# NoliNobdon/TriStage-RAG

Hardware: AMD Instinct MI355X
Metric: end-to-end queries/sec @10Mx768 corpus (stage-1 exact top-k, pre-encoded HBM-resident queries) (higher is better)
Workload: dtype f16; 1 GPU; synthetic 10000000x768 f16 corpus, batch-64 queries, stage-1 exact top-1000, row-sharded over 1 GPU(s); rows=10000000, dim=768, batch=64, k=1000, submission=batches enqueued back to back (async), verified by finish() in the timed region, max_candidates_per_query=6027

## Files before the change

include/tristage.h:

```cpp
#ifndef TRISTAGE_H_
#define TRISTAGE_H_

#include <stdint.h>

#ifdef __cplusplus
extern "C" {
#endif

#define TS_ABI_VERSION 4

typedef struct ts_index ts_index;

enum ts_status {
  TS_OK = 0,
  TS_ERR_INVALID = -1,
  TS_ERR_HIP = -2,
  TS_ERR_OOM = -3,
  TS_ERR_EMPTY = -4,
  TS_ERR_UNSUPPORTED = -5
};

enum ts_dtype { TS_F32 = 0, TS_F16 = 1, TS_BF16 = 2,
               TS_FP8_E4M3 = 3  };

enum ts_metric { TS_METRIC_INNER_PRODUCT = 0 };

#define TS_FLAG_HOST_PTR 1u
#define TS_FLAG_NO_FILTER 2u
#define TS_FLAG_ASYNC 8u
#define TS_FLAG_PIPELINE 16u
#define TS_FLAG_CLASSIC 32u
#define TS_FLAG_ONE_LAUNCH 64u
#define TS_FLAG_COALESCE 128u
#define TS_FLAG_WIDE_PASSES 256u
#define TS_FLAG_NO_WIDE_PASSES 512u
#define TS_FLAG_NORMALIZE 4u

int ts_index_create(int32_t dim, int32_t storage_dtype, int32_t metric,
                    int32_t device, ts_index** out);
int ts_index_destroy(ts_index* h);
int ts_index_reset(ts_index* h);
int ts_index_reserve(ts_index* h, int64_t nrows);

int ts_index_add(ts_index* h, const void* rows, int64_t n, int32_t rows_dtype,
                 uint32_t flags, void* stream);

int ts_index_search(ts_index* h, const void* queries, int32_t nq,
                    int32_t q_dtype, int32_t k, float* out_scores,
                    int64_t* out_ids, uint32_t flags, void* stream);

int ts_index_search_filtered(ts_index* h, const void* queries, int32_t nq, int32_t q_dtype, int32_t k,
                             const uint32_t* allow_bits, int64_t allow_words, int32_t n_masks,
                             const int32_t* mask_of_query, float* out_scores, int64_t* out_ids,
                             uint32_t flags, void* stream);
int ts_index_last_filter_info(const ts_index* h, int64_t info[4]);

int ts_index_range_search(ts_index* h, const void* queries, int32_t nq, int32_t q_dtype, const float* radius,
                          const uint32_t* allow_bits, int64_t allow_words, int32_t n_masks,
                          const int32_t* mask_of_query, int64_t max_total, int64_t* lims, uint32_t flags,
                          void* stream);
int ts_index_range_fetch(ts_index* h, float* out_scores, int64_t* out_ids, int64_t capacity, uint32_t flags,
                         void* stream);

int ts_index_scores(ts_index* h, const void* queries, int32_t nq, int32_t q_dtype,
                    float* out, int64_t ld, void* stream);

int64_t ts_index_last_ticket(const ts_index* h);
int ts_index_filter_path(const ts_index* h, int32_t k);
int ts_index_finish(ts_index* h, void* stream, int64_t* failed_tickets, int32_t max_failed,
                    int32_t* n_failed);

int ts_index_flush(ts_index* h, void* stream);
int32_t ts_coalesce_groups(int32_t dim, int32_t storage_dtype);
int32_t ts_coalesce_groups_wide(int32_t dim, int32_t storage_dtype);
int64_t ts_coalesce_wide_min_bytes(void);

int ts_index_remove(ts_index* h, const int64_t* ids, int64_t n, int64_t* n_removed, void* stream);
int64_t ts_index_live_count(const ts_index* h);
int ts_index_live_words(ts_index* h, uint32_t* out, void* stream);
int ts_index_compact(ts_index* h, int64_t* old2new, void* stream);

int ts_index_update(ts_index* h, const int64_t* ids, int64_t n, const void* rows, int32_t rows_dtype,
                    uint32_t flags, void* stream);

int64_t ts_index_ntotal(const ts_index* h);
int32_t ts_index_dim(const ts_index* h);
int32_t ts_index_dtype(const ts_index* h);

int ts_index_set_fp8_scale_log2(ts_index* h, int32_t s);
int32_t ts_index_fp8_scale_log2(const ts_index* h);
int ts_index_mmr(ts_index* h, const int64_t* cand_ids, const float* cand_rel, int32_t nq, int32_t fetch_k, int32_t k,
                 float lambda, float* out_rel, int64_t* out_ids, uint32_t flags, void* stream);
int ts_index_mmr_set_timing(ts_index* h, int32_t on);
int ts_index_mmr_get_timings(ts_index* h, double ms[3], int64_t* calls, int32_t reset);
int ts_index_search_prefix(ts_index* h, const void* queries, int32_t nq, int32_t q_dtype, int32_t dims, int32_t k,
                           const uint32_t* allow_bits, int64_t allow_words, int32_t n_masks,
                           const int32_t* mask_of_query, float* out_scores, int64_t* out_ids, uint32_t flags,
                           void* hip_stream);
int ts_index_rescore(ts_index* h, const void* queries, int32_t nq, int32_t q_dtype, const int64_t* cand_ids,
                     int32_t ncand, int32_t k, float* out_scores, int64_t* out_ids, void* hip_stream);
int ts_index_set_id_offset(ts_index* h, int64_t offset);
int ts_index_reconstruct(ts_index* h, int64_t row0, int64_t n, float* out,
                         uint32_t flags, void* stream);
int ts_index_last_search_info(const ts_index* h, int64_t info[4]);

int ts_index_set_profiling(ts_index* h, int32_t on);
int ts_index_get_timings(ts_index* h, double ms[8], int64_t counts[8], int32_t reset);

// ... 142 lines not shown
```

tristage-rag_amd/_lib.py:

```python
from __future__ import annotations

import ctypes
import os
import subprocess
from ctypes import POINTER, c_char_p, c_float, c_int32, c_int64, c_uint32, c_void_p

_HERE = os.path.dirname(os.path.abspath(__file__))
LIB_PATH = os.environ.get("TRISTAGE_LIB") or os.path.join(_HERE, "libtristage.so")
CSRC_DIR = os.path.join(_HERE, "csrc")

TS_OK = 0
TS_ERR_INVALID, TS_ERR_HIP, TS_ERR_OOM, TS_ERR_EMPTY, TS_ERR_UNSUPPORTED = -1, -2, -3, -4, -5
TS_F32, TS_F16, TS_BF16, TS_FP8_E4M3 = 0, 1, 2, 3
TS_METRIC_INNER_PRODUCT = 0
HEADER_PATH = os.path.join(os.path.dirname(_HERE), "include", "tristage.h")


def header_abi_version() -> int:
    import re
    m = re.search(r"^#define\s+TS_ABI_VERSION\s+(\d+)", open(HEADER_PATH).read(), flags=re.M)
    if not m:
        raise ImportError(f"TS_ABI_VERSION not found in {HEADER_PATH}")
    return int(m.group(1))


TS_FLAG_HOST_PTR, TS_FLAG_NO_FILTER, TS_FLAG_NORMALIZE, TS_FLAG_ASYNC, TS_FLAG_PIPELINE, TS_FLAG_CLASSIC, TS_FLAG_ONE_LAUNCH = 1, 2, 4, 8, 16, 32, 64
TS_FLAG_COALESCE = 128
TS_FLAG_WIDE_PASSES, TS_FLAG_NO_WIDE_PASSES = 256, 512

SIGNATURES = {
    "ts_index_create": (c_int32, [c_int32, c_int32, c_int32, c_int32, POINTER(c_void_p)]),
    "ts_index_destroy": (c_int32, [c_void_p]),
    "ts_index_reset": (c_int32, [c_void_p]),
    "ts_index_reserve": (c_int32, [c_void_p, c_int64]),
    "ts_index_add": (c_int32, [c_void_p, c_void_p, c_int64, c_int32, c_uint32, c_void_p]),
    "ts_index_search": (c_int32, [c_void_p, c_void_p, c_int32, c_int32, c_int32, c_void_p,
                                  c_void_p, c_uint32, c_void_p]),
    "ts_index_search_filtered": (c_int32, [c_void_p, c_void_p, c_int32, c_int32, c_int32, c_void_p, c_int64, c_int32,
                                           c_void_p, c_void_p, c_void_p, c_uint32, c_void_p]),
    "ts_index_last_filter_info": (c_int32, [c_void_p, POINTER(c_int64)]),
    "ts_index_range_search": (c_int32, [c_void_p, c_void_p, c_int32, c_int32, c_void_p, c_void_p, c_int64, c_int32,
                                        c_void_p, c_int64, c_void_p, c_uint32, c_void_p]),
    "ts_index_range_fetch": (c_int32, [c_void_p, c_void_p, c_void_p, c_int64, c_uint32, c_void_p]),
    "ts_index_scores": (c_int32, [c_void_p, c_void_p, c_int32, c_int32, c_void_p, c_int64, c_void_p]),
    "ts_index_remove": (c_int32, [c_void_p, c_void_p, c_int64, POINTER(c_int64), c_void_p]),
    "ts_index_update": (c_int32, [c_void_p, c_void_p, c_int64, c_void_p, c_int32, c_uint32, c_void_p]),
    "ts_index_live_count": (c_int64, [c_void_p]),
    "ts_index_live_words": (c_int32, [c_void_p, c_void_p, c_void_p]),
    "ts_index_compact": (c_int32, [c_void_p, c_void_p, c_void_p]),
    "ts_index_ntotal": (c_int64, [c_void_p]),
    "ts_index_dim": (c_int32, [c_void_p]),
    "ts_index_dtype": (c_int32, [c_void_p]),
    "ts_index_set_fp8_scale_log2": (c_int32, [c_void_p, c_int32]),
    "ts_index_fp8_scale_log2": (c_int32, [c_void_p]),
    "ts_index_set_id_offset": (c_int32, [c_void_p, c_int64]),
    "ts_index_reconstruct": (c_int32, [c_void_p, c_int64, c_int64, c_void_p, c_uint32, c_void_p]),
    "ts_index_last_search_info": (c_int32, [c_void_p, POINTER(c_int64)]),
    "ts_index_last_ticket": (c_int64, [c_void_p]),
    "ts_index_filter_path": (c_int32, [c_void_p, c_int32]),
    "ts_index_finish": (c_int32, [c_void_p, c_void_p, POINTER(c_int64), c_int32, POINTER(c_int32)]),
    "ts_index_flush": (c_int32, [c_void_p, c_void_p]),
    "ts_coalesce_groups": (c_int32, [c_int32, c_int32]),
    "ts_coalesce_groups_wide": (c_int32, [c_int32, c_int32]),
    "ts_coalesce_wide_min_bytes": (c_int64, []),
    "ts_index_set_profiling": (c_int32, [c_void_p, c_int32]),
    "ts_index_get_timings": (c_int32, [c_void_p, POINTER(ctypes.c_double), POINTER(c_int64), c_int32]),
    "ts_index_read_probe": (c_int32, [c_void_p, c_int32, POINTER(ctypes.c_double), POINTER(ctypes.c_double),
                                      POINTER(c_int64), c_void_p]),
    "ts_ivf_create": (c_int32, [c_int32, c_int32, c_int32, c_int32, POINTER(c_void_p)]),
    "ts_ivf_destroy": (c_int32, [c_void_p]),
    "ts_ivf_reset": (c_int32, [c_void_p]),
    "ts_ivf_train": (c_int32, [c_void_p, c_void_p, c_int64, c_int32, c_int64, c_int32, c_void_p, c_void_p]),
    "ts_ivf_set_centroids": (c_int32, [c_void_p, c_void_p, c_void_p]),
    "ts_ivf_get_centroids": (c_int32, [c_void_p, c_void_p, c_void_p]),
    "ts_ivf_is_trained": (c_int32, [c_void_p]),
    "ts_ivf_add": (c_int32, [c_void_p, c_void_p, c_int64, c_int32, c_uint32, c_void_p]),
    "ts_ivf_search": (c_int32, [c_void_p, c_void_p, c_int32, c_int32, c_int32, c_int32, c_void_p, c_void_p, c_void_p]),
    "ts_ivf_probe": (c_int32, [c_void_p, c_void_p, c_int32, c_int32, c_int32, c_void_p, c_void_p, c_void_p]),
    "ts_ivf_list_sizes": (c_int32, [c_void_p, c_void_p]),
    "ts_ivf_reconstruct": (c_int32, [c_void_p, c_int64, c_int64, c_void_p, c_void_p]),
    "ts_ivf_ntotal": (c_int64, [c_void_p]),
    "ts_remove_ivf": (c_int32, [c_void_p, c_void_p, c_int64, POINTER(c_int64), c_void_p]),
    "ts_update_ivf": (c_int32, [c_void_p, c_void_p, c_int64, c_void_p, c_int32, c_uint32, c_void_p]),
    "ts_compact_ivf": (c_int32, [c_void_p, c_void_p, c_void_p]),
    "ts_index_mmr": (c_int32, [c_void_p, c_void_p, c_void_p, c_int32, c_int32, c_int32, c_float, c_void_p, c_void_p,
                               c_uint32, c_void_p]),
    "ts_index_search_prefix": (c_int32, [c_void_p, c_void_p, c_int32, c_int32, c_int32, c_int32, c_void_p, c_int64, c_int32,
                                         c_void_p, c_void_p, c_void_p, c_uint32, c_void_p]),
    "ts_index_rescore": (c_int32, [c_void_p, c_void_p, c_int32, c_int32, c_void_p, c_int32, c_int32, c_void_p, c_void_p,
                                   c_void_p]),
    "ts_index_mmr_set_timing": (c_int32, [c_void_p, c_int32]),
    "ts_index_mmr_get_timings": (c_int32, [c_void_p, POINTER(ctypes.c_double), POINTER(c_int64), c_int32]),
    "ts_mmr_ivf": (c_int32, [c_void_p, c_void_p, c_void_p, c_int32, c_int32, c_int32, c_float, c_void_p, c_void_p,
                             c_uint32, c_void_p]),
    "ts_ivf_set_id_offset": (c_int32, [c_void_p, c_int64]),
    "ts_ivf_last_search_info": (c_int32, [c_void_p, POINTER(c_int64)]),
# ... 108 lines not shown
```

tristage-rag_amd/csrc/ts_common.h:

```cpp
#pragma once
#include <hip/hip_runtime.h>
#include <stdint.h>
#include <stddef.h>

#include "../../include/tristage.h"

void ts_set_error(const char* fmt, ...);

#define TS_HIP(call)                                                        \
  do {                                                                      \
    hipError_t e_ = (call);                                                 \
    if (e_ != hipSuccess) {                                                 \
      ts_set_error("%s failed: %s (%s:%d)", #call, hipGetErrorString(e_),   \
                   __FILE__, __LINE__);                                     \
      return (e_ == hipErrorOutOfMemory) ? TS_ERR_OOM : TS_ERR_HIP;         \
    }                                                                       \
  } while (0)

#define TS_CHECK(call)            \
  do {                            \
    int s_ = (call);              \
    if (s_ != TS_OK) return s_;   \
  } while (0)

// ... 102 lines not shown
                                 hipStream_t stream);

#define TS_MAX_GROUPS 4
struct MultiScanParams : ScanParams {
  const uint4* gimg[TS_MAX_GROUPS];
  int gqh[TS_MAX_GROUPS];
  int ghalf[TS_MAX_GROUPS];
  const float* gtau[TS_MAX_GROUPS];
  uint32_t* gcnt[TS_MAX_GROUPS];
  float* gscore[TS_MAX_GROUPS];
  int32_t* gid[TS_MAX_GROUPS];
  uint32_t stage_cap;
};
int ts_scan_multi_groups(const TsLayout& L);
uint32_t ts_scan_multi_stage_cap(const TsLayout& L, int G);
bool ts_scan_multi_fits(int64_t nblk, int num_cus);
int ts_launch_scan_multi(const TsLayout& L, int G, const MultiScanParams& p, int num_cus, hipStream_t stream);

#define TS_MAX_WIDE_GROUPS 8
struct WideScanParams : ScanParams {
  const uint4* gimg[TS_MAX_WIDE_GROUPS];
  int gqh[TS_MAX_WIDE_GROUPS];
  int ghalf[TS_MAX_WIDE_GROUPS];
  const float* gtau[TS_MAX_WIDE_GROUPS];
  uint32_t* gcnt[TS_MAX_WIDE_GROUPS];
  float* gscore[TS_MAX_WIDE_GROUPS];
  int32_t* gid[TS_MAX_WIDE_GROUPS];
  uint32_t stage_cap;
};
int ts_scan_wide_groups(const TsLayout& L);
uint32_t ts_scan_wide_stage_cap(const TsLayout& L, int G);
bool ts_scan_wide_fits(int64_t nblk, int num_cus);
int ts_launch_scan_wide(const TsLayout& L, int G, const WideScanParams& p, int num_cus, hipStream_t stream);

struct MultiTombParams : MultiScanParams {
  const uint32_t* live;
};
struct WideTombParams : WideScanParams {
  const uint32_t* live;
};
int ts_launch_scan_multi_tomb(const TsLayout& L, int G, const MultiTombParams& p, int num_cus, hipStream_t stream);
int ts_launch_scan_wide_tomb(const TsLayout& L, int G, const WideTombParams& p, int num_cus, hipStream_t stream);

int ts_launch_scan(const TsLayout& L, int mode, int qh, const ScanParams& p,
                   int num_cus, hipStream_t stream);

struct TsMaskPass {
  int32_t nd;
  int32_t all_live;
  int32_t dist[TS_MAX_Q];
  int32_t qmask[TS_MAX_Q];
  int32_t qd[TS_MAX_Q];
};
struct TsMaskDev {
  int32_t qmask[TS_MAX_Q];
  int32_t qd[TS_MAX_Q];
  uint32_t popc[TS_MAX_Q];
  uint32_t need[TS_MAX_Q];
  uint32_t nlive;
  uint32_t pad[63];
};
int ts_launch_live_blocks(const uint32_t* bits, int64_t words, const TsMaskPass& mp, int64_t nblk,
                          int64_t ntotal, TsMaskDev* md, hipStream_t stream);
int ts_launch_tau_masked(const float* sample, int64_t S, int64_t sstride, int64_t ntotal, const uint32_t* bits,
                         int64_t words, TsMaskDev* md, int nq, int k, uint32_t over, uint32_t min_rank,
                         float* tau, uint32_t* report, hipStream_t stream);
// ... 214 lines not shown
```

tristage-rag_amd/csrc/ts_index.hip:

```cpp
#include <stdarg.h>
#include <stdio.h>
#include <string.h>
#include <stdlib.h>

#include <algorithm>
#include <atomic>
#include <condition_variable>
#include <mutex>
#include <new>
#include <thread>
#include <vector>

#include "ts_common.h"

static thread_local char g_err[512] = "";

void ts_set_error(const char* fmt, ...) {
  va_list ap;
  va_start(ap, fmt);
  vsnprintf(g_err, sizeof(g_err), fmt, ap);
  va_end(ap);
}

extern "C" const char* ts_last_error(void) { return g_err; }
// ... 32 lines not shown
    b.p = nullptr;
    ts_set_error("hipMalloc(%zu bytes) failed: %s", want, hipGetErrorString(e));
    return TS_ERR_OOM;
  }
  b.bytes = want;
  return TS_OK;
}

void release(DevBuf& b) {
  if (b.p) (void)hipFree(b.p);
  b.p = nullptr;
  b.bytes = 0;
}

}
#define TS_NPHASE 8
#define TS_NSETS 8
#define TS_ASYNC_SLOTS 1024
#define TS_SLOT_WORDS 80
namespace {
constexpr int64_t kMinFilterRows = 32768;
constexpr int kMaxFilterK = 2048;
constexpr uint32_t kCandCap = 16384;
constexpr int64_t kMinSampleRows = 8192;
constexpr int64_t kSampleDiv = 128;
constexpr uint32_t kMinSampleRank = 24;
constexpr uint32_t kOversample = 4;
constexpr int64_t kDenseChunkRows = 1 << 20;
constexpr int64_t kOneLaunchMaxRows = 4 << 20;
constexpr int kHeadStartUs = 12;
constexpr int64_t kCoalesceOversample = 3;
constexpr int64_t kWideMinCorpusBytes = 256ll << 20;
constexpr int kWideMaxResidentGroups = 3;

}

struct ts_index {
  int device = 0;
  int num_cus = 256;
  TsLayout L{};
  int64_t ntotal = 0;
  int64_t cap_blocks = 0;
  uint4* corpus = nullptr;
  int64_t id_offset = 0;
  int64_t info[4] = {0, 0, 0, 0};
  int64_t finfo[4] = {0, 0, 0, 0};
  int64_t fseq = 0;
  struct WSet {
    DevBuf qimg, small, cand_score, cand_id, sample;
    DevBuf dense, list_score, list_id;
    DevBuf hist, spill;
    DevBuf mask, mids;
    uint32_t gen = 0;
    uint32_t arrive_total = 0;
    bool hist_dirty = false;
    unsigned long long* tau64() { return (unsigned long long*)((char*)small.p + 1024); }
    uint32_t* arrive() { return (uint32_t*)((char*)small.p + 2048); }
    hipEvent_t ev_pro = nullptr, ev_scan = nullptr, ev_sel = nullptr, ev_in = nullptr;
    bool used = false;
    bool busy = false;
    float* tau() { return (float*)small.p; }
    uint32_t* cand_cnt() { return (uint32_t*)small.p + 64; }
    uint32_t* status() { return (uint32_t*)small.p + 128; }
  };
  WSet ws[TS_NSETS];
  uint64_t set_next = 0;
  std::mutex mu;
  std::condition_variable cv;
  std::mutex host_mu;
  std::mutex prof_mu;
  bool slot_busy[TS_ASYNC_SLOTS] = {};
  hipStream_t s_pro = nullptr, s_scan = nullptr, s_sel = nullptr;
  DevBuf stage, den, qstage, out_s, out_i, mstage;
  uint32_t* host_status = nullptr;
  uint32_t* host_status_dev = nullptr;
  struct Pending { int64_t ticket; int slot; int nq; uint32_t S; uint32_t m; hipEvent_t e0, e1; int set; int64_t fseq; };
  Pending pending[TS_ASYNC_SLOTS];
  int npending = 0;
  uint64_t slot_next = 0;
  int64_t next_ticket = 0;
  hipEvent_t async_ev[2 * TS_ASYNC_SLOTS] = {};
  struct CoBatch { WSet* W; int nq, qh, k, slot, groups_left; float* out_s; int64_t* out_i; };
  struct CoGroup { int batch, half; };
  std::mutex co_mu;
  int co_gmax = 0;
  int co_gwide = 0;
  int co_width = 0;
  hipStream_t co_stream = nullptr;
  CoBatch co_batch[TS_MAX_WIDE_GROUPS] = {};
  int co_nbatch = 0;
  CoGroup co_group[TS_MAX_WIDE_GROUPS] = {};
  int co_ngroup = 0;
  uint64_t co_pass_seq = 0;
  hipEvent_t co_ev = nullptr;
  bool co_ev_live = false;
  bool profiling = false;
  int prof_every = 1;
  std::atomic<uint64_t> prof_seq{0};
  hipEvent_t ev[TS_NPHASE + 1] = {};
  double phase_ms[TS_NPHASE] = {};
  int64_t phase_cnt[TS_NPHASE] = {};
  DevBuf live;
  int64_t live_cap_words = 0;
  int64_t nremoved = 0;
  DevBuf eff, rids, compact_scratch, compact_stage;
  DevBuf upd_tile, upd_tab;
  std::mutex eff_mu;
  hipEvent_t eff_ev = nullptr;
  bool eff_used = false;
  DevBuf rng_s, rng_i, rng_tiles;
  int64_t rng_cap = 0, rng_total = 0;
  bool rng_valid = false;
  std::mutex range_mu;
  TsMmrWork mmr;
  DevBuf rescore_scratch;
  std::mutex rescore_mu;
};

static int co_flush(ts_index* h, hipStream_t s);

// ... 53 lines not shown
                               int32_t device, ts_index** out) {
  if (!out) { ts_set_error("out is null"); return TS_ERR_INVALID; }
  *out = nullptr;
  if (dim <= 0 || dim > 65536) { ts_set_error("bad dim %d", dim); return TS_ERR_INVALID; }
  if (storage_dtype != TS_F32 && storage_dtype != TS_F16 && storage_dtype != TS_BF16 &&
      storage_dtype != TS_FP8_E4M3) {
    ts_set_error("bad storage dtype %d", storage_dtype);
    return TS_ERR_INVALID;
  }
  if (metric != TS_METRIC_INNER_PRODUCT) {
    ts_set_error("only the inner-product metric is supported (reference uses IndexFlatIP)");
    return TS_ERR_UNSUPPORTED;
  }
  int ndev = 0;
  TS_HIP(hipGetDeviceCount(&ndev));
  if (device < 0 || device >= ndev) {
    ts_set_error("device %d not present (%d HIP devices)", device, ndev);
    return TS_ERR_INVALID;
  }
  TsLayout L = ts_make_layout(dim, storage_dtype);
  if (ts_scan_lds_bytes(L, 1) > 160 * 1024) {
    ts_set_error("dim %d with dtype %d needs %zu bytes of LDS for 32 queries (max 163840)", dim,
                 storage_dtype, ts_scan_lds_bytes(L, 1));
    return TS_ERR_UNSUPPORTED;
  }
  DeviceGuard g(device);
  if (!g.ok) { ts_set_error("hipSetDevice(%d) failed", device); return TS_ERR_HIP; }
  ts_index* h = new (std::nothrow) ts_index();
  if (!h) { ts_set_error("out of host memory"); return TS_ERR_OOM; }
  h->device = device;
  h->L = L;
  h->co_gmax = ts_coalesce_groups(dim, storage_dtype);
  h->co_gwide = ts_coalesce_groups_wide(dim, storage_dtype);
  hipDeviceProp_t prop;
  if (hipGetDeviceProperties(&prop, device) == hipSuccess && prop.multiProcessorCount > 0)
    h->num_cus = prop.multiProcessorCount;
  int st = TS_OK;
  for (ts_index::WSet& w : h->ws) {
    if (st == TS_OK) st = ensure(w.small, 4096);
    if (st == TS_OK && hipMemset(w.small.p, 0, 4096) != hipSuccess) { ts_set_error("hipMemset failed"); st = TS_ERR_HIP; }
    if (st == TS_OK) st = ensure(w.qimg, (size_t)L.qkg * 2 * 1024);
    if (st == TS_OK && (hipEventCreateWithFlags(&w.ev_pro, hipEventDisableTiming) != hipSuccess ||
                        hipEventCreateWithFlags(&w.ev_scan, hipEventDisableTiming) != hipSuccess ||
                        hipEventCreateWithFlags(&w.ev_sel, hipEventDisableTiming) != hipSuccess ||
                        hipEventCreateWithFlags(&w.ev_in, hipEventDisableTiming) != hipSuccess)) {
      ts_set_error("hipEventCreate failed");
      st = TS_ERR_HIP;
    }
  }
  if (st == TS_OK && hipStreamSynchronize(nullptr) != hipSuccess) { ts_set_error("hipStreamSynchronize failed"); st = TS_ERR_HIP; }
  if (st == TS_OK && (hipEventCreateWithFlags(&h->co_ev, hipEventDisableTiming) != hipSuccess ||
                      hipEventCreateWithFlags(&h->eff_ev, hipEventDisableTiming) != hipSuccess)) {
    ts_set_error("hipEventCreate failed");
    st = TS_ERR_HIP;
  }
  if (st == TS_OK &&
      (hipHostMalloc((void**)&h->host_status, (size_t)(TS_ASYNC_SLOTS + 1) * TS_SLOT_WORDS * 4, hipHostMallocMapped) != hipSuccess ||
       hipHostGetDevicePointer((void**)&h->host_status_dev, h->host_status, 0) != hipSuccess)) {
    ts_set_error("hipHostMalloc(mapped) failed");
    st = TS_ERR_HIP;
  }
  if (st != TS_OK) {
    ts_index_destroy(h);
    return st;
  }
  *out = h;
  return TS_OK;
}

extern "C" int ts_index_destroy(ts_index* h) {
// ... 676 lines not shown
  TS_HIP(hipStreamSynchronize(s));
  prof_collect(h, pc);
  uint32_t maxc = 0;
  for (int i = 0; i < nq; ++i) maxc = std::max(maxc, rep[i]);
  const bool redo = rep[64] != 0;
  set_info(h, (redo ? 2 : 1) | (fused ? 16 : 0), maxc, S, m);
  if (mc) add_filter_info(h, fseq, rep[65], nblk, false);
  if (redo) {
    if (fused) {
      W.hist_dirty = true;
      TS_CHECK(ts_launch_qprep(h->L, dq, q_dtype, nq, qh, (uint4*)W.qimg.p, W.cand_cnt(), W.status(), s));
    }
    prof_mark(h, pc, 5, s);
    TS_CHECK(dense_path(h, W, nq, qh, k, out_s, out_i, s, mc, pkg));
    prof_mark(h, pc, -1, s);
    TS_HIP(hipStreamSynchronize(s));
    prof_collect(h, pc);
  }
  return TS_OK;
}

extern "C" int32_t ts_coalesce_groups(int32_t dim, int32_t storage_dtype) {
  if (dim <= 0 || (storage_dtype != TS_F16 && storage_dtype != TS_BF16)) return 0;
  return ts_scan_multi_groups(ts_make_layout(dim, storage_dtype));
}

extern "C" int32_t ts_coalesce_groups_wide(int32_t dim, int32_t storage_dtype) {
  if (dim <= 0 || (storage_dtype != TS_F16 && storage_dtype != TS_BF16)) return 0;
  return ts_scan_wide_groups(ts_make_layout(dim, storage_dtype));
}

extern "C" int64_t ts_coalesce_wide_min_bytes() { return kWideMinCorpusBytes; }

static int co_pass_width(const ts_index* h, int k, uint32_t flags) {
  const int64_t N = h->ntotal;
  const int64_t nblk = (N + TS_ROWS_PER_BLOCK - 1) / TS_ROWS_PER_BLOCK;
  const uint32_t need = TS_FLAG_ASYNC | TS_FLAG_COALESCE;
  if ((flags & need) != need || (flags & (TS_FLAG_PIPELINE | TS_FLAG_NO_FILTER | TS_FLAG_HOST_PTR | TS_FLAG_ONE_LAUNCH)))
    return 0;
  if (k > kMaxFilterK || N < kMinFilterRows || N < 32 * (int64_t)k) return 0;
  if (!(flags & TS_FLAG_CLASSIC) && N <= kOneLaunchMaxRows) return 0;
  const int grid = h->num_cus - h->num_cus / 8;
  bool wide = (int64_t)nblk * (int64_t)ts_block_bytes(h->L) > kWideMinCorpusBytes &&
              h->co_gmax <= kWideMaxResidentGroups;
  if (flags & TS_FLAG_WIDE_PASSES) wide = true;
  if (flags & TS_FLAG_NO_WIDE_PASSES) wide = false;
  if (wide && h->co_gwide >= 3 && ts_scan_wide_fits(nblk, h->num_cus)) return h->co_gwide;
  if (h->co_gmax >= 3 && ts_scan_multi_fits(nblk, grid)) return h->co_gmax;
  return 0;
}

template <class P>
static void co_fill_params(const ts_index* h, int G, P& mp) {
  const int64_t N = h->ntotal;
  mp.corpus = h->corpus;
  mp.kg = h->L.kg;
  mp.nwork = (N + TS_ROWS_PER_BLOCK - 1) / TS_ROWS_PER_BLOCK;
  mp.blk0 = 0;
  mp.blk_stride = 1;
  mp.ntotal = N;
  mp.cand_cap = kCandCap;
  for (int g = 0; g < G; ++g) {
    const ts_index::CoBatch& b = h->co_batch[h->co_group[g].batch];
    const int half = h->co_group[g].half;
    mp.gimg[g] = (const uint4*)b.W->qimg.p;
    mp.gqh[g] = b.qh;
    mp.ghalf[g] = half;
    mp.gtau[g] = b.W->tau() + 32 * half;
    mp.gcnt[g] = b.W->cand_cnt() + 32 * half;
    mp.gscore[g] = (float*)b.W->cand_score.p + (size_t)32 * half * kCandCap;
    mp.gid[g] = (int32_t*)b.W->cand_id.p + (size_t)32 * half * kCandCap;
  }
}

static int co_launch_pass(ts_index* h) {
  if (h->co_ngroup == 0) return TS_OK;
  const int G = h->co_ngroup;
  const int64_t N = h->ntotal;
  hipStream_t s = h->co_stream;
  hipEvent_t e0 = nullptr, e1 = nullptr;
  if (h->profiling && h->co_pass_seq++ % (uint64_t)h->prof_every == 0) {
    if (hipEventCreate(&e0) != hipSuccess || hipEventCreate(&e1) != hipSuccess || hipEventRecord(e0, s) != hipSuccess) {
      if (e0) (void)hipEventDestroy(e0);
      if (e1) (void)hipEventDestroy(e1);
      e0 = e1 = nullptr;
    }
  }
  int st;
  const bool tomb = h->nremoved > 0;
  if (G <= h->co_gmax) {
    MultiTombParams mp{};
    co_fill_params(h, G, mp);
    mp.stage_cap = ts_scan_multi_stage_cap(h->L, G);
    mp.live = (const uint32_t*)h->live.p;
    st = tomb ? ts_launch_scan_multi_tomb(h->L, G, mp, h->num_cus - h->num_cus / 8, s)
              : ts_launch_scan_multi(h->L, G, mp, h->num_cus - h->num_cus / 8, s);
  } else {
    WideTombParams wp{};
    co_fill_params(h, G, wp);
    wp.stage_cap = ts_scan_wide_stage_cap(h->L, G);
    wp.live = (const uint32_t*)h->live.p;
    int wide_cus = h->num_cus;
#ifdef TS_TUNING
    static const int dbg_wide_cus = getenv("TS_WIDE_CUS") ? atoi(getenv("TS_WIDE_CUS")) : 0;
    if (dbg_wide_cus > 0) wide_cus = dbg_wide_cus;
#endif
    st = tomb ? ts_launch_scan_wide_tomb(h->L, G, wp, wide_cus, s) : ts_launch_scan_wide(h->L, G, wp, wide_cus, s);
  }
  if (e0 && (st != TS_OK || hipEventRecord(e1, s) != hipSuccess)) {
    (void)hipEventDestroy(e0);
    (void)hipEventDestroy(e1);
    e0 = e1 = nullptr;
  }
  for (int g = 0; g < G; ++g) --h->co_batch[h->co_group[g].batch].groups_left;
  h->co_ngroup = 0;
  int keep = 0;
  const int nb = h->co_nbatch;
  for (int i = 0; i < nb; ++i) {
    ts_index::CoBatch b = h->co_batch[i];
    if (b.groups_left > 0) { h->co_batch[keep++] = b; continue; }
    if (st == TS_OK) {
      SelParams p{};
      p.mode = SEL_PAIRS32;
// ... 156 lines not shown
    std::vector<int32_t> moq((size_t)nq, -1);
    return ts_index_search_filtered(h, queries, nq, q_dtype, k, nullptr, 0, 0, moq.data(), out_scores, out_ids, flags,
                                    stream);
  }
  DeviceGuard g(h->device);
  hipStream_t s = (hipStream_t)stream;
  const int qp = (ts_scan_lds_bytes(h->L, 2) <= 160 * 1024) ? 64 : 32;
  if ((flags & TS_FLAG_PIPELINE) && !(flags & TS_FLAG_ASYNC)) {
    ts_set_error("TS_FLAG_PIPELINE needs TS_FLAG_ASYNC");
    return TS_ERR_INVALID;
  }
  if (flags & TS_FLAG_ASYNC) {
    if (flags & TS_FLAG_HOST_PTR) { ts_set_error("TS_FLAG_ASYNC needs device pointers"); return TS_ERR_INVALID; }
    const int passes = (nq + qp - 1) / qp;
    if (passes > 4) { ts_set_error("TS_FLAG_ASYNC: at most %d queries per call", 4 * qp); return TS_ERR_INVALID; }
    bool full = false;
    {
      std::lock_guard<std::mutex> lk(h->mu);
      full = h->npending + passes > TS_ASYNC_SLOTS / 4;
    }
    if (full) {
      (void)co_flush(h, s);
      ts_set_error("too many unfinished asynchronous searches; call ts_index_finish()");
      return TS_ERR_INVALID;
    }
  }
  const size_t qrow = (size_t)h->L.dim * dtype_size(q_dtype);
  if (const int width = co_pass_width(h, k, flags)) {
    std::lock_guard<std::mutex> lk(h->co_mu);
    if (h->co_stream != s) TS_CHECK(co_flush_locked(h, s));
    if (h->co_ngroup > 0 && h->co_width != width) TS_CHECK(co_flush_locked(h, s));
    h->co_stream = s;
    h->co_width = width;
    for (int q0 = 0; q0 < nq; q0 += qp) {
      const int c = std::min(qp, nq - q0);
      TS_CHECK(co_submit(h, (const char*)queries + (size_t)q0 * qrow, c, q_dtype, k, out_scores + (size_t)q0 * k,
                         out_ids + (size_t)q0 * k, s));
    }
    std::lock_guard<std::mutex> lk2(h->mu);
    ++h->next_ticket;
    return TS_OK;
  }
  TS_CHECK(co_flush(h, s));
  const void* dq = queries;
  float* ds = out_scores;
  int64_t* di = out_ids;
  const bool host = (flags & TS_FLAG_HOST_PTR) != 0;
  std::unique_lock<std::mutex> hlk(h->host_mu, std::defer_lock);
  if (host) {
    hlk.lock();
    TS_CHECK(ensure(h->qstage, (size_t)nq * qrow));
    TS_CHECK(ensure(h->out_s, (size_t)nq * k * 4));
    TS_CHECK(ensure(h->out_i, (size_t)nq * k * 8));
    TS_HIP(hipMemcpyAsync(h->qstage.p, queries, (size_t)nq * qrow, hipMemcpyHostToDevice, s));
    dq = h->qstage.p;
    ds = (float*)h->out_s.p;
    di = (int64_t*)h->out_i.p;
  }
  for (int q0 = 0; q0 < nq; q0 += qp) {
    const int c = std::min(qp, nq - q0);
    TS_CHECK(search_pass(h, (const char*)dq + (size_t)q0 * qrow, c, q_dtype, k,
                         ds + (size_t)q0 * k, di + (size_t)q0 * k, flags, s));
  }
  if (flags & TS_FLAG_ASYNC) {
    std::lock_guard<std::mutex> lk(h->mu);
    ++h->next_ticket;
// ... 1319 lines not shown
```

tristage-rag_amd/index.py:

```python
from __future__ import annotations

import ctypes
from typing import NamedTuple, Optional

import numpy as np

from . import _lib

_NP_DTYPES = {np.dtype(np.float32): _lib.TS_F32, np.dtype(np.float16): _lib.TS_F16}
_NAME_TO_DTYPE = {"f32": _lib.TS_F32, "fp32": _lib.TS_F32, "float32": _lib.TS_F32,
                  "f16": _lib.TS_F16, "fp16": _lib.TS_F16, "float16": _lib.TS_F16,
                  "bf16": _lib.TS_BF16, "bfloat16": _lib.TS_BF16,
                  "fp8": _lib.TS_FP8_E4M3, "e4m3": _lib.TS_FP8_E4M3, "float8_e4m3fn": _lib.TS_FP8_E4M3}
_DTYPE_NAME = {_lib.TS_F32: "f32", _lib.TS_F16: "f16", _lib.TS_BF16: "bf16", _lib.TS_FP8_E4M3: "fp8"}
FP8_INDEX_MAX_D = 2048


def _torch():
    import torch
    return torch


def _is_tensor(x) -> bool:
    return type(x).__module__.startswith("torch") and hasattr(x, "data_ptr")
# ... 15 lines not shown
        mask = mask.detach().cpu().numpy()
    m = np.asarray(mask)
    words = (int(n) + 31) // 32
    if m.dtype == np.bool_:
        if m.ndim != 1 or m.shape[0] != n:
            raise ValueError(f"a bool allow mask must have one entry per row ({n}), got shape {m.shape}")
        b = np.packbits(m, bitorder="little")
        out = np.zeros(words * 4, dtype=np.uint8)
        out[: b.shape[0]] = b
        return out.view("<u4").astype(np.uint32)
    if m.dtype in (np.uint32, np.int32):
        if m.ndim != 1 or m.shape[0] < words:
            raise ValueError(f"a packed allow mask needs >= {words} uint32 words, got shape {m.shape}")
        w = np.ascontiguousarray(m[:words]).view(np.uint32).copy()
        if n % 32:
            w[-1] &= np.uint32((1 << (n % 32)) - 1)
        return w
    raise TypeError(f"allow mask: expected a bool array or packed uint32 words, got dtype {m.dtype}")


def _stream_ptr(device_index: int) -> int:
    torch = _torch()
    return int(torch.cuda.current_stream(device_index).cuda_stream)


def wide_pass_flags(wide_passes) -> int:
    if wide_passes is True:
        return _lib.TS_FLAG_WIDE_PASSES
    if wide_passes is False:
        return _lib.TS_FLAG_NO_WIDE_PASSES
    if isinstance(wide_passes, str) and wide_passes == "auto":
        return 0
    raise ValueError(f"wide_passes must be 'auto', True or False, not {wide_passes!r}")


def _addr(x) -> Optional[int]:
    if x is None:
        return None
    return x.data_ptr() if _is_tensor(x) else x.ctypes.data


def _raise_empty():
    raise ValueError("No documents indexed. Call add_documents() first.")


def _check(code: int, invalid: bool = False) -> None:
    if code == _lib.TS_ERR_EMPTY:
        _raise_empty()
    if invalid and code == _lib.TS_ERR_INVALID:
        raise ValueError(_lib.last_error())
    _lib.check(code)



def _bad_shape(n, d: int, what: str, shape):
    raise ValueError(f"expected [{n}, {d}] {what}, got {tuple(shape)}")


def _host_query(x, d: int, what: str = "queries", n="B", device: Optional[int] = None):
    if _is_tensor(x) and not x.is_cuda:
        x = x.detach().float().numpy()
    on_gpu = _is_tensor(x)
    if not on_gpu:
        x = np.ascontiguousarray(x)
        if x.dtype not in _NP_DTYPES:
            x = x.astype(np.float32)
# ... 307 lines not shown

    supports_out = True
    PENDING_PASSES = 240
    MAX_KERNEL_K = 16384
    MAX_ASYNC_QUERIES = 128

    def __init__(self, d: int, dtype: str = "f32", device: int = 0, fp8_scale_log2: int = 8):
        if dtype not in _NAME_TO_DTYPE:
            raise ValueError(f"unknown storage dtype {dtype!r}")
        is_fp8 = _NAME_TO_DTYPE[dtype] == _lib.TS_FP8_E4M3
        if is_fp8 and not 0 <= int(fp8_scale_log2) <= 15:
            raise ValueError(f"fp8_scale_log2 must be in 0 .. 15, got {fp8_scale_log2}")
        if is_fp8 and int(d) > FP8_INDEX_MAX_D:
            raise NotImplementedError(f"an fp8 index takes at most {FP8_INDEX_MAX_D} dimensions, got {d}")
        self._lib = _lib.load()
        self.d = int(d)
        self.device = int(device)
        self.storage_dtype = _DTYPE_NAME[_NAME_TO_DTYPE[dtype]]
        self._h = ctypes.c_void_p()
        _lib.check(self._lib.ts_index_create(self.d, _NAME_TO_DTYPE[dtype],
                                             _lib.TS_METRIC_INNER_PRODUCT, self.device,
                                             ctypes.byref(self._h)))
        if is_fp8:
            self.set_fp8_scale_log2(fp8_scale_log2)
        self.is_trained = True
        self._pending = {}
        self._pending_passes = 0
        self._auto_redone = []
        self.auto_finish = True
        self.classic_filter = False
        self.one_launch_filter = False
        self.coalesce = True
        self.wide_passes = "auto"
        self._filter_info = None

    @property
    def ntotal(self) -> int:
        return int(self._lib.ts_index_ntotal(self._h))

    def train(self, x) -> None:
        return None

    @property
    def nlive(self) -> int:
        return int(self._lib.ts_index_live_count(self._h))

    def remove_ids(self, ids) -> int:
        arr = _id_array(ids)
        self._finish_pending()
        n = ctypes.c_int64(0)
        _lib.check(self._lib.ts_index_remove(self._h, _addr(arr), int(arr.shape[0]), ctypes.byref(n),
                                             _stream_ptr(self.device)))
        return int(n.value)

    def _finish_pending(self) -> None:
        if self._pending:
            self._auto_redone = self._auto_redone + self.finish()

    def update_rows(self, ids, x, normalize: bool = False) -> None:
        arr = _id_array(ids)
        x, dt, _, on_gpu = _host_query(x, self.d, "rows", int(arr.shape[0]), self.device)
        flags = (_lib.TS_FLAG_NORMALIZE if normalize else 0) | (0 if on_gpu else _lib.TS_FLAG_HOST_PTR)
        self._finish_pending()
        _update_call(self._lib.ts_index_update, self._h, arr, x, dt, flags, _stream_ptr(self.device))

    def live_words(self) -> np.ndarray:
# ... 42 lines not shown
            raise ValueError("k must be positive")
        if allowed is not None and self.ntotal == 0:
            _raise_empty()
        if k > self.MAX_KERNEL_K and self.ntotal > self.MAX_KERNEL_K:
            return self._search_large_k(q, k, out, allowed)
        if async_ and not (_is_tensor(q) and q.is_cuda):
            raise ValueError("async_ search needs a CUDA tensor")
        q, q_dtype, B, on_gpu = _host_query(q, self.d)
        D, I = _outputs(out if on_gpu else None, B, k, q)
        if async_ and B > self.MAX_ASYNC_QUERIES:
            items = None if allowed is None else _allowed_items(allowed, B)
            for s in range(0, B, self.MAX_ASYNC_QUERIES):
                e = min(B, s + self.MAX_ASYNC_QUERIES)
                self.search(q[s:e], k, exact_dense=exact_dense, async_=True, out=(D[s:e], I[s:e]),
                            inputs_ready=inputs_ready, classic=classic, one_launch=one_launch,
                            allowed=None if items is None else items[s:e])
            return D, I
        flags = (_lib.TS_FLAG_NO_FILTER if exact_dense else 0) | (0 if on_gpu else _lib.TS_FLAG_HOST_PTR)
        stream = _stream_ptr(self.device) if on_gpu else None
        masks = None
        if allowed is None:
            if classic or self.classic_filter:
                flags |= _lib.TS_FLAG_CLASSIC
            elif one_launch or self.one_launch_filter:
                flags |= _lib.TS_FLAG_ONE_LAUNCH
            if async_:
                self._admit_async(B)
                flags |= _lib.TS_FLAG_ASYNC
                if inputs_ready:
                    flags |= _lib.TS_FLAG_PIPELINE
                elif self.coalesce:
                    flags |= _lib.TS_FLAG_COALESCE
                    flags |= wide_pass_flags(self.wide_passes)
            self._search_raw(q, q_dtype, k, D, I, flags, stream)
        else:
            self._filter_info = None
            masks = _marshal_allowed(allowed, B, self.ntotal, q.device if on_gpu else None)
            if async_:
                self._admit_async(B)
                flags |= _lib.TS_FLAG_ASYNC
            self._filtered_raw(q, q_dtype, k, masks, D, I, flags, stream)
        if async_:
            self._pending[int(self._lib.ts_index_last_ticket(self._h))] = (q, k, D, I, masks)
            self._pending_passes += (B + 31) // 32
        return D, I

    def _admit_async(self, n_queries: int) -> None:
        if self.pending_room(n_queries) < 0:
            if not self.auto_finish:
                raise RuntimeError("too many unfinished asynchronous searches: the owner of this index "
                                   "must call finish() (see pending_room())")
            self._auto_redone = self.finish()

    def _search_raw(self, q, q_dtype: int, k: int, D, I, flags: int, stream) -> None:
        _check(self._lib.ts_index_search(self._h, _addr(q), q.shape[0], q_dtype, k, _addr(D), _addr(I), flags, stream))

    def _filtered_raw(self, q, q_dtype: int, k: int, m: _Masks, D, I, flags: int, stream) -> None:
        _check(self._lib.ts_index_search_filtered(self._h, _addr(q), q.shape[0], q_dtype, k, _addr(m.keep), m.words,
                                                  m.n_masks, _addr(m.moq), _addr(D), _addr(I), flags, stream))

    def _search_large_k(self, q, k: int, out, allowed):
        torch = _torch()
        if not (_is_tensor(q) and q.is_cuda):
            q = np.ascontiguousarray(_to_host(q.float() if _is_tensor(q) else q), dtype=np.float32)
        qt, _, B, on_gpu = _device_query(q, self.d, self.device)
        n = self.ntotal
# ... 936 lines not shown
```

Baseline: 56710 queries/s.

## Add query-stationary coalesced scan kernel with async LDS-ring corpus streaming

Adds a new scan kernel that keeps each wave's 32-query group resident in registers (query-stationary) while corpus blocks stream into a multi-slot LDS ring via global_load_lds with explicit vmcnt waits. Survivors above each query's threshold are staged in LDS and bucketed per query before a single global atomic reservation per query. It becomes the default path for large, untombstoned f16/bf16 corpora when auto wide passes would apply. The aim is to stream the corpus once for up to eight groups with fewer global atomics. The cost is heavy LDS use, hand-written inline asm, and risk of staging overflow falling back to global atomics.

```diff
diff --git a/include/tristage.h b/include/tristage.h
--- a/include/tristage.h
+++ b/include/tristage.h
@@ -34,6 +34,8 @@
 #define TS_FLAG_COALESCE 128u
 #define TS_FLAG_WIDE_PASSES 256u
 #define TS_FLAG_NO_WIDE_PASSES 512u
+#define TS_FLAG_STATIONARY_PASSES 1024u
+#define TS_FLAG_NO_STATIONARY_PASSES 2048u
 #define TS_FLAG_NORMALIZE 4u
 
 int ts_index_create(int32_t dim, int32_t storage_dtype, int32_t metric,
@@ -74,6 +76,7 @@
 int32_t ts_coalesce_groups(int32_t dim, int32_t storage_dtype);
 int32_t ts_coalesce_groups_wide(int32_t dim, int32_t storage_dtype);
 int64_t ts_coalesce_wide_min_bytes(void);
+int32_t ts_coalesce_groups_stationary(int32_t dim, int32_t storage_dtype);
 
 int ts_index_remove(ts_index* h, const int64_t* ids, int64_t n, int64_t* n_removed, void* stream);
 int64_t ts_index_live_count(const ts_index* h);
diff --git a/tristage-rag_amd/_lib.py b/tristage-rag_amd/_lib.py
--- a/tristage-rag_amd/_lib.py
+++ b/tristage-rag_amd/_lib.py
@@ -27,6 +27,7 @@
 TS_FLAG_HOST_PTR, TS_FLAG_NO_FILTER, TS_FLAG_NORMALIZE, TS_FLAG_ASYNC, TS_FLAG_PIPELINE, TS_FLAG_CLASSIC, TS_FLAG_ONE_LAUNCH = 1, 2, 4, 8, 16, 32, 64
 TS_FLAG_COALESCE = 128
 TS_FLAG_WIDE_PASSES, TS_FLAG_NO_WIDE_PASSES = 256, 512
+TS_FLAG_STATIONARY_PASSES, TS_FLAG_NO_STATIONARY_PASSES = 1024, 2048
 
 SIGNATURES = {
     "ts_index_create": (c_int32, [c_int32, c_int32, c_int32, c_int32, POINTER(c_void_p)]),
@@ -62,6 +63,7 @@
     "ts_index_flush": (c_int32, [c_void_p, c_void_p]),
     "ts_coalesce_groups": (c_int32, [c_int32, c_int32]),
     "ts_coalesce_groups_wide": (c_int32, [c_int32, c_int32]),
+    "ts_coalesce_groups_stationary": (c_int32, [c_int32, c_int32]),
     "ts_coalesce_wide_min_bytes": (c_int64, []),
     "ts_index_set_profiling": (c_int32, [c_void_p, c_int32]),
     "ts_index_get_timings": (c_int32, [c_void_p, POINTER(ctypes.c_double), POINTER(c_int64), c_int32]),
diff --git a/tristage-rag_amd/csrc/ts_common.h b/tristage-rag_amd/csrc/ts_common.h
--- a/tristage-rag_amd/csrc/ts_common.h
+++ b/tristage-rag_amd/csrc/ts_common.h
@@ -158,6 +158,12 @@
 uint32_t ts_scan_wide_stage_cap(const TsLayout& L, int G);
 bool ts_scan_wide_fits(int64_t nblk, int num_cus);
 int ts_launch_scan_wide(const TsLayout& L, int G, const WideScanParams& p, int num_cus, hipStream_t stream);
+
+int ts_scan_qstat_groups(const TsLayout& L);
+uint32_t ts_scan_qstat_stage_cap(const TsLayout& L);
+bool ts_scan_qstat_fits(int64_t nblk, int num_cus);
+int ts_scan_qstat_prepare(const TsLayout& L);
+int ts_launch_scan_qstat(const TsLayout& L, int G, const WideScanParams& p, int num_cus, hipStream_t stream);
 
 struct MultiTombParams : MultiScanParams {
   const uint32_t* live;
diff --git a/tristage-rag_amd/csrc/ts_index.hip b/tristage-rag_amd/csrc/ts_index.hip
--- a/tristage-rag_amd/csrc/ts_index.hip
+++ b/tristage-rag_amd/csrc/ts_index.hip
@@ -88,6 +88,7 @@
 constexpr int64_t kCoalesceOversample = 3;
 constexpr int64_t kWideMinCorpusBytes = 256ll << 20;
 constexpr int kWideMaxResidentGroups = 3;
+constexpr bool kStationaryByDefault = true;
 
 }
 
@@ -141,7 +142,9 @@
   std::mutex co_mu;
   int co_gmax = 0;
   int co_gwide = 0;
+  int co_gstat = 0;
   int co_width = 0;
+  bool co_stat_forced = false;
   hipStream_t co_stream = nullptr;
   CoBatch co_batch[TS_MAX_WIDE_GROUPS] = {};
   int co_nbatch = 0;
@@ -261,10 +264,11 @@
   h->L = L;
   h->co_gmax = ts_coalesce_groups(dim, storage_dtype);
   h->co_gwide = ts_coalesce_groups_wide(dim, storage_dtype);
+  h->co_gstat = ts_coalesce_groups_stationary(dim, storage_dtype);
   hipDeviceProp_t prop;
   if (hipGetDeviceProperties(&prop, device) == hipSuccess && prop.multiProcessorCount > 0)
     h->num_cus = prop.multiProcessorCount;
-  int st = TS_OK;
+  int st = ts_scan_qstat_prepare(L);
   for (ts_index::WSet& w : h->ws) {
     if (st == TS_OK) st = ensure(w.small, 4096);
     if (st == TS_OK && hipMemset(w.small.p, 0, 4096) != hipSuccess) { ts_set_error("hipMemset failed"); st = TS_ERR_HIP; }
@@ -1007,6 +1011,11 @@
 
 extern "C" int64_t ts_coalesce_wide_min_bytes() { return kWideMinCorpusBytes; }
 
+extern "C" int32_t ts_coalesce_groups_stationary(int32_t dim, int32_t storage_dtype) {
+  if (dim <= 0 || (storage_dtype != TS_F16 && storage_dtype != TS_BF16)) return 0;
+  return ts_scan_qstat_groups(ts_make_layout(dim, storage_dtype));
+}
+
 static int co_pass_width(const ts_index* h, int k, uint32_t flags) {
   const int64_t N = h->ntotal;
   const int64_t nblk = (N + TS_ROWS_PER_BLOCK - 1) / TS_ROWS_PER_BLOCK;
@@ -1018,6 +1027,11 @@
   const int grid = h->num_cus - h->num_cus / 8;
   bool wide = (int64_t)nblk * (int64_t)ts_block_bytes(h->L) > kWideMinCorpusBytes &&
               h->co_gmax <= kWideMaxResidentGroups;
+  if (h->co_gstat > 0 && h->nremoved == 0 && !(flags & TS_FLAG_NO_STATIONARY_PASSES) &&
+      ts_scan_qstat_fits(nblk, h->num_cus)) {
+    const bool auto_wide = wide && !(flags & (TS_FLAG_WIDE_PASSES | TS_FLAG_NO_WIDE_PASSES));
+    if ((flags & TS_FLAG_STATIONARY_PASSES) || (kStationaryByDefault && auto_wide)) return h->co_gstat;
+  }
   if (flags & TS_FLAG_WIDE_PASSES) wide = true;
   if (flags & TS_FLAG_NO_WIDE_PASSES) wide = false;
   if (wide && h->co_gwide >= 3 && ts_scan_wide_fits(nblk, h->num_cus)) return h->co_gwide;
@@ -1063,7 +1077,18 @@
   }
   int st;
   const bool tomb = h->nremoved > 0;
-  if (G <= h->co_gmax) {
+  const int stat_above = h->co_stat_forced ? h->co_gmax : std::max(h->co_gmax, h->co_gwide);
+  if (!tomb && h->co_gstat > 0 && h->co_width == h->co_gstat && G > stat_above) {
+    WideScanParams wp{};
+    co_fill_params(h, G, wp);
+    wp.stage_cap = ts_scan_qstat_stage_cap(h->L);
+    int stat_cus = h->num_cus;
+#ifdef TS_TUNING
+    static const int dbg_stat_cus = getenv("TS_QSTAT_CUS") ? atoi(getenv("TS_QSTAT_CUS")) : 0;
+    if (dbg_stat_cus > 0) stat_cus = dbg_stat_cus;
+#endif
+    st = ts_launch_scan_qstat(h->L, G, wp, stat_cus, s);
+  } else if (G <= h->co_gmax) {
     MultiTombParams mp{};
     co_fill_params(h, G, mp);
     mp.stage_cap = ts_scan_multi_stage_cap(h->L, G);
@@ -1286,6 +1311,7 @@
     if (h->co_ngroup > 0 && h->co_width != width) TS_CHECK(co_flush_locked(h, s));
     h->co_stream = s;
     h->co_width = width;
+    h->co_stat_forced = (flags & TS_FLAG_STATIONARY_PASSES) != 0;
     for (int q0 = 0; q0 < nq; q0 += qp) {
       const int c = std::min(qp, nq - q0);
       TS_CHECK(co_submit(h, (const char*)queries + (size_t)q0 * qrow, c, q_dtype, k, out_scores + (size_t)q0 * k,
diff --git a/tristage-rag_amd/csrc/ts_scan_qstat.hip b/tristage-rag_amd/csrc/ts_scan_qstat.hip
--- /dev/null
+++ b/tristage-rag_amd/csrc/ts_scan_qstat.hip
@@ -0,0 +1,275 @@
+#include "ts_scan_dev.h"
+#include "ts_linear_dev.h"
+#include <algorithm>
+#include <type_traits>
+
+struct StageQstatHdr {
+  uint32_t cnt;
+  uint32_t pad[3];
+  uint32_t qcnt[TS_MAX_WIDE_GROUPS * 32];
+  uint32_t qbase[TS_MAX_WIDE_GROUPS * 32];
+  uint32_t qoff[TS_MAX_WIDE_GROUPS * 32];
+};
+static_assert(SCAN_WAVES == 8 && TS_MAX_WIDE_GROUPS == SCAN_WAVES, "one group per wave");
+static_assert(TS_RING == SCAN_WAVES, "a window is one piece per wave");
+#define TS_QSTAT_GROUPS 8
+#define TS_QSTAT_MAX_STEPS (1 << 16)
+#define TS_QSTAT_MIN_STAGE 4096u
+#define TS_QSTAT_WINDOW 8192u
+#define TS_QSTAT_DEPTH 15
+#define TS_QSTAT_AHEAD 4
+#define TS_QSTAT_MAX_LEAD 8
+
+template <class T>
+__device__ __forceinline__ T qstat_pick(const T (&a)[TS_MAX_WIDE_GROUPS], int g) {
+  T r = a[0];
+#pragma unroll
+  for (int i = 1; i < TS_MAX_WIDE_GROUPS; ++i) r = (g == i) ? a[i] : r;
+  return r;
+}
+
+template <int N, int I = 0, class F>
+__device__ __forceinline__ void qstat_static_for(F&& f) {
+  if constexpr (I < N) {
+    f(std::integral_constant<int, I>{});
+    qstat_static_for<N, I + 1>(f);
+  }
+}
+
+__device__ __forceinline__ void qstat_wait_vm(int n) {
+  switch (n) {
+    case 0: __builtin_amdgcn_s_waitcnt(0x3F70 | 0); break;
+    case 1: __builtin_amdgcn_s_waitcnt(0x3F70 | 1); break;
+    case 2: __builtin_amdgcn_s_waitcnt(0x3F70 | 2); break;
+    case 3: __builtin_amdgcn_s_waitcnt(0x3F70 | 3); break;
+    case 4: __builtin_amdgcn_s_waitcnt(0x3F70 | 4); break;
+    case 5: __builtin_amdgcn_s_waitcnt(0x3F70 | 5); break;
+    case 6: __builtin_amdgcn_s_waitcnt(0x3F70 | 6); break;
+    case 7: __builtin_amdgcn_s_waitcnt(0x3F70 | 7); break;
+    default: __builtin_amdgcn_s_waitcnt(0x3F70 | 8); break;
+  }
+}
+
+template <int DT, int NWIN>
+__global__ __launch_bounds__(SCAN_THREADS) void scan_qstat_kernel(WideScanParams p, int G, int depth) {
+  extern __shared__ __attribute__((aligned(16))) unsigned char smem[];
+  constexpr int KG = NWIN * TS_RING;
+  const int tid = threadIdx.x;
+  const int lane = tid & 63;
+  const int wave = __builtin_amdgcn_readfirstlane(tid >> 6);
+  const bool owner = wave < G;
+  const int grid = (int)gridDim.x;
+  const int steps = (int)((p.nwork - 1 - (int64_t)blockIdx.x) / grid) + 1;
+
+  StageQstatHdr* st = reinterpret_cast<StageQstatHdr*>(smem + (size_t)depth * TS_QSTAT_WINDOW);
+  float* sscore = reinterpret_cast<float*>(st + 1);
+  uint32_t* skey = reinterpret_cast<uint32_t*>(sscore + p.stage_cap);
+  if (tid == 0) st->cnt = 0;
+
+  const unsigned char* corpus = reinterpret_cast<const unsigned char*>(p.corpus);
+  const size_t blk_bytes = (size_t)KG * 1024;
+  const uint32_t loff = (uint32_t)lane * 16;
+  const uint32_t ring_lds = (uint32_t)(uintptr_t)(__attribute__((address_space(3))) void*)smem + (uint32_t)wave * 1024u;
+  const unsigned char* const dead = reinterpret_cast<const unsigned char*>(p.gimg[0]) + (size_t)wave * 1024;
+  auto blk_of = [&](int s) { return p.blk0 + ((int64_t)blockIdx.x + (int64_t)s * grid) * p.blk_stride; };
+  int fstep = 0, fkw = 0, fslot = 0;
+  const unsigned char* fsrc = corpus + (size_t)blk_of(0) * blk_bytes + (size_t)wave * 1024;
+  auto request = [&]() {
+    const unsigned char* src = fstep < steps ? fsrc : dead;
+    const uint32_t dst = ring_lds + (uint32_t)fslot * TS_QSTAT_WINDOW;
+    uint32_t keep;
+    __asm__ volatile("s_nop 4\n\ts_mov_b32 %0, m0\n\ts_mov_b32 m0, %3\n\ts_nop 0\n\t"
+                     "global_load_lds_dwordx4 %1, %2 nt\n\ts_mov_b32 m0, %0"
+                     : "=&s"(keep) : "v"(loff), "s"(src), "s"(dst) : "memory");
+    fslot = fslot + 1 == depth ? 0 : fslot + 1;
+    if (++fkw == NWIN) {
+      fkw = 0;
+      ++fstep;
+      if (fstep < steps) fsrc = corpus + (size_t)blk_of(fstep) * blk_bytes + (size_t)wave * 1024;
+    } else {
+      fsrc += TS_QSTAT_WINDOW;
+    }
+  };
+  for (int i = 0; i < depth; ++i) request();
+
+  const int gqh = qstat_pick(p.gqh, wave), ghalf = qstat_pick(p.ghalf, wave);
+  u32x4 q[KG];
+  float tau = __builtin_huge_valf();
+  if (owner) {
+    const u32x4* img = reinterpret_cast<const u32x4*>(qstat_pick(p.gimg, wave)) + (size_t)ghalf * 64 + lane;
+#pragma unroll
+    for (int i = 0; i < KG; ++i) q[i] = img[(size_t)i * gqh * 64];
+    tau = qstat_pick(p.gtau, wave)[lane & 31];
+  } else {
+#pragma unroll
+    for (int i = 0; i < KG; ++i) q[i] = u32x4{0u, 0u, 0u, 0u};
+  }
+#pragma unroll
+  for (int i = 0; i < KG; ++i) __asm__ volatile("" : "+v"(q[i]));
+  __asm__ volatile("" : "+v"(tau));
+  __builtin_amdgcn_s_waitcnt(0x3F70);
+  fs_barrier();
+
+  const int lead = depth - 2 * NWIN;
+  int slot0 = 0;
+
+  auto survivors = [&](const f32x16& acc, int sb) {
+    if (__builtin_amdgcn_ballot_w64(acc_max(acc) >= tau) == 0ull) return;
+    const int64_t row_base = blk_of(sb) * TS_ROWS_PER_BLOCK;
+    const bool partial = row_base + TS_ROWS_PER_BLOCK > p.ntotal;
+    const int rows_left = (int)(p.ntotal - row_base);
+    const uint32_t keyhi = (uint32_t)sb << 16;
+#pragma unroll
+    for (int r = 0; r < 16; ++r) {
+      const bool ok = acc[r] >= tau;
+      if (__builtin_expect(__builtin_amdgcn_ballot_w64(ok) == 0ull, 1)) continue;
+      if (!ok) continue;
+      int ln = lane;
+      __asm__ volatile("" : "+v"(ln));
+      const int row = acc_row(r, ln), j = ln & 31;
+      if (!partial || row < rows_left) {
+        const uint32_t slot = atomicAdd(&st->cnt, 1u);
+        if (slot < p.stage_cap) {
+          sscore[slot] = acc[r];
+          skey[slot] = keyhi | ((uint32_t)row << 8) | (uint32_t)(wave * 32 + j);
+        } else {
+          const uint32_t g = atomicAdd(&qstat_pick(p.gcnt, wave)[j], 1u);
+          if (g < p.cand_cap) {
+            qstat_pick(p.gscore, wave)[(size_t)j * p.cand_cap + g] = acc[r];
+            qstat_pick(p.gid, wave)[(size_t)j * p.cand_cap + g] = (int32_t)(row_base + row);
+          }
+        }
+      }
+    }
+  };
+
+  for (int s = 0; s < steps; ++s) {
+    if (owner) {
+      uint32_t woff[NWIN];
+#pragma unroll
+      for (int kw = 0; kw < NWIN; ++kw) {
+        int sl = slot0 + kw;
+        sl = sl >= depth ? sl - depth : sl;
+        woff[kw] = (uint32_t)sl * TS_QSTAT_WINDOW + loff;
+      }
+      auto a_read = [&](auto i) {
+        constexpr int I = decltype(i)::value;
+        return *reinterpret_cast<const u32x4*>(smem + woff[I / TS_RING] + (I % TS_RING) * 1024);
+      };
+      u32x4 a[TS_QSTAT_AHEAD];
+      qstat_static_for<TS_QSTAT_AHEAD>([&](auto i) { a[decltype(i)::value] = a_read(i); });
+      f32x16 acc;
+#pragma unroll
+      for (int r = 0; r < 16; ++r) acc[r] = 0.f;
+      __builtin_amdgcn_sched_barrier(0);
+      qstat_static_for<KG>([&](auto i) {
+        constexpr int I = decltype(i)::value;
+        mma_group<DT>(acc, a[I % TS_QSTAT_AHEAD], q[I]);
+        __builtin_amdgcn_sched_barrier(0);
+        if constexpr (I + TS_QSTAT_AHEAD < KG) {
+          a[I % TS_QSTAT_AHEAD] = a_read(std::integral_constant<int, I + TS_QSTAT_AHEAD>{});
+          __builtin_amdgcn_sched_barrier(0);
+        }
+      });
+      survivors(acc, s);
+    }
+    qstat_wait_vm(lead);
+    fs_barrier();
+#pragma unroll
+    for (int kw = 0; kw < NWIN; ++kw) request();
+    slot0 += NWIN;
+    slot0 = slot0 >= depth ? slot0 - depth : slot0;
+  }
+  __builtin_amdgcn_s_waitcnt(0x3F70);
+
+  __syncthreads();
+  const uint32_t n = st->cnt < p.stage_cap ? st->cnt : p.stage_cap;
+  if (n == 0) return;
+  for (int t = tid; t < TS_QSTAT_GROUPS * 32; t += SCAN_THREADS) { st->qcnt[t] = 0; st->qoff[t] = 0; }
+  __syncthreads();
+  for (uint32_t e = tid; e < n; e += SCAN_THREADS) atomicAdd(&st->qcnt[skey[e] & 255u], 1u);
+  __syncthreads();
+  for (int t = tid; t < TS_QSTAT_GROUPS * 32; t += SCAN_THREADS)
+    if (st->qcnt[t] > 0) st->qbase[t] = atomicAdd(qstat_pick(p.gcnt, t >> 5) + (t & 31), st->qcnt[t]);
+  __syncthreads();
+  for (uint32_t e = tid; e < n; e += SCAN_THREADS) {
+    const uint32_t key = skey[e];
+    const uint32_t qi = key & 255u;
+    const uint32_t slot = st->qbase[qi] + atomicAdd(&st->qoff[qi], 1u);
+    if (slot < p.cand_cap) {
+      const int g = (int)(qi >> 5);
+      const size_t at = (size_t)(qi & 31u) * p.cand_cap + slot;
+      const int64_t wi = (int64_t)blockIdx.x + (int64_t)(key >> 16) * grid;
+      qstat_pick(p.gscore, g)[at] = sscore[e];
+      qstat_pick(p.gid, g)[at] = (int32_t)((p.blk0 + wi * p.blk_stride) * TS_ROWS_PER_BLOCK + ((key >> 8) & 31u));
+    }
+  }
+}
+
+static int qstat_nwin(const TsLayout& L) {
+  if (L.dtype != TS_F16 && L.dtype != TS_BF16) return 0;
+  const int nwin = L.kg / TS_RING;
+  return (L.kg % TS_RING == 0 && (nwin == 5 || nwin == 6)) ? nwin : 0;
+}
+
+static int qstat_depth(const TsLayout& L) {
+  const int depth = TS_QSTAT_DEPTH;
+  const int nwin = qstat_nwin(L);
+  return std::max(2 * nwin, std::min(depth, 2 * nwin + TS_QSTAT_MAX_LEAD));
+}
+
+int ts_scan_qstat_groups(const TsLayout& L) {
+  return qstat_nwin(L) > 0 && ts_scan_qstat_stage_cap(L) > 0 ? TS_QSTAT_GROUPS : 0;
+}
+
+uint32_t ts_scan_qstat_stage_cap(const TsLayout& L) {
+  if (qstat_nwin(L) == 0) return 0;
+  const size_t fixed = (size_t)qstat_depth(L) * TS_QSTAT_WINDOW + sizeof(StageQstatHdr);
+  if (fixed + 8 * (size_t)TS_QSTAT_MIN_STAGE > 160 * 1024) return 0;
+  return (uint32_t)((160 * 1024 - fixed) / 8);
+}
+
+bool ts_scan_qstat_fits(int64_t nblk, int num_cus) {
+  const int64_t grid = std::max<int64_t>(1, std::min<int64_t>(nblk, num_cus));
+  return (nblk + grid - 1) / grid <= TS_QSTAT_MAX_STEPS;
+}
+
+template <int DT, int NWIN>
+static int qstat_kernel_t(const WideScanParams* p, int G, int depth, size_t lds, int grid, hipStream_t stream) {
+  void (*kern)(WideScanParams, int, int) = scan_qstat_kernel<DT, NWIN>;
+  static TsDeviceOnce lds_attr;
+  TS_CHECK(ts_allow_max_lds(lds_attr, reinterpret_cast<const void*>(kern)));
+  if (!p) return TS_OK;
+  hipLaunchKernelGGL(kern, dim3(grid), dim3(SCAN_THREADS), lds, stream, *p, G, depth);
+  TS_HIP(hipGetLastError());
+  return TS_OK;
+}
+
+static int qstat_dispatch(const TsLayout& L, const WideScanParams* p, int G, int depth, size_t lds, int grid,
+                          hipStream_t stream) {
+  const int nwin = qstat_nwin(L);
+  if (L.dtype == TS_F16 && nwin == 5) return qstat_kernel_t<TS_F16, 5>(p, G, depth, lds, grid, stream);
+  if (L.dtype == TS_F16 && nwin == 6) return qstat_kernel_t<TS_F16, 6>(p, G, depth, lds, grid, stream);
+  if (L.dtype == TS_BF16 && nwin == 5) return qstat_kernel_t<TS_BF16, 5>(p, G, depth, lds, grid, stream);
+  if (L.dtype == TS_BF16 && nwin == 6) return qstat_kernel_t<TS_BF16, 6>(p, G, depth, lds, grid, stream);
+  ts_set_error("stationary scan: no kernel for dtype %d at dimension %d", L.dtype, L.dim);
+  return TS_ERR_UNSUPPORTED;
+}
+
+int ts_scan_qstat_prepare(const TsLayout& L) {
+  if (ts_scan_qstat_groups(L) == 0) return TS_OK;
+  return qstat_dispatch(L, nullptr, 0, 0, 0, 0, nullptr);
+}
+
+int ts_launch_scan_qstat(const TsLayout& L, int G, const WideScanParams& p, int num_cus, hipStream_t stream) {
+  if (p.nwork <= 0) return TS_OK;
+  if (G < 1 || G > TS_QSTAT_GROUPS || ts_scan_qstat_groups(L) == 0 || p.kg != L.kg || p.stage_cap == 0 ||
+      p.stage_cap > ts_scan_qstat_stage_cap(L) || !ts_scan_qstat_fits(p.nwork, num_cus)) {
+    ts_set_error("stationary scan: %d groups do not fit at dimension %d", G, L.dim);
+    return TS_ERR_UNSUPPORTED;
+  }
+  const int depth = qstat_depth(L);
+  const size_t lds = (size_t)depth * TS_QSTAT_WINDOW + sizeof(StageQstatHdr) + 8 * (size_t)p.stage_cap;
+  const int grid = (int)std::max<int64_t>(1, std::min<int64_t>(p.nwork, num_cus));
+  return qstat_dispatch(L, &p, G, depth, lds, grid, stream);
+}
diff --git a/tristage-rag_amd/index.py b/tristage-rag_amd/index.py
--- a/tristage-rag_amd/index.py
+++ b/tristage-rag_amd/index.py
@@ -71,6 +71,16 @@
     if isinstance(wide_passes, str) and wide_passes == "auto":
         return 0
     raise ValueError(f"wide_passes must be 'auto', True or False, not {wide_passes!r}")
+
+
+def stationary_pass_flags(stationary_passes) -> int:
+    if stationary_passes is True:
+        return _lib.TS_FLAG_STATIONARY_PASSES
+    if stationary_passes is False:
+        return _lib.TS_FLAG_NO_STATIONARY_PASSES
+    if isinstance(stationary_passes, str) and stationary_passes == "auto":
+        return 0
+    raise ValueError(f"stationary_passes must be 'auto', True or False, not {stationary_passes!r}")
 
 
 def _addr(x) -> Optional[int]:
@@ -444,6 +454,7 @@
         self.one_launch_filter = False
         self.coalesce = True
         self.wide_passes = "auto"
+        self.stationary_passes = "auto"
         self._filter_info = None
 
     @property
@@ -552,6 +563,7 @@
                 elif self.coalesce:
                     flags |= _lib.TS_FLAG_COALESCE
                     flags |= wide_pass_flags(self.wide_passes)
+                    flags |= stationary_pass_flags(self.stationary_passes)
             self._search_raw(q, q_dtype, k, D, I, flags, stream)
         else:
             self._filter_info = None
```

After: 58610 queries/s, median of 6. 3.4% higher.
